# irap-omp/deconv3d

Measured on AMD Instinct MI355X. Metric: spaxel-updates/sec (MH-Gibbs), higher is better.
Workload: dtype f64; 1 GPU; c3_300x300x128; fsf=moffat 11x11, lsf_taps=17, spaxels=90000, lsf=analytic MUSE stand-in (mpdaf absent), parallelism=1 chain, variance=per-voxel cube (heteroscedastic)

## Files before the change

__graft_entry__.py:

```python
import os
import subprocess
import sys

ROOT = os.path.dirname(os.path.abspath(__file__))
if ROOT not in sys.path:
    sys.path.insert(0, ROOT)
CSRC = os.path.join(ROOT, "deconv3d_amd", "csrc")


SOURCES = ["d3d_api.hip", "d3d_spatial.hip", "d3d_mh.hip", "d3d_sweep.hip", "d3d_post.hip", "d3d_region.hip", "d3d_search.hip", "d3d_prep.hip", "d3d_temper.hip", "d3d_robust.hip", "d3d_pred.hip", "d3d_noise.hip", "d3d_ctx.h", "d3d_kernels.h", "d3d_conv.h",
           "d3d_mh_small.h", "d3d_rng.h", "../../include/deconv3d_hip.h", "d3d_strips.h"]


def tree_source_hash():
    import hashlib
    h = hashlib.sha256()
    for name in SOURCES:
        with open(os.path.join(CSRC, name), "rb") as f:
            h.update(f.read())
    return h.hexdigest()[:16]


def _binary_hash(lib):
    code = ("import ctypes,sys; l=ctypes.CDLL(sys.argv[1]); "
            "l.d3d_source_hash.restype=ctypes.c_char_p; print(l.d3d_source_hash().decode())")
    try:
        return subprocess.check_output([sys.executable, "-c", code, lib],
                                       stderr=subprocess.DEVNULL).decode().strip()
    except (subprocess.CalledProcessError, OSError):
        return None


def build():
    env = dict(os.environ)
    lib = os.path.join(CSRC, "libdeconv3d_hip.so")
    want = tree_source_hash()
    have = _binary_hash(lib) if os.path.exists(lib) else None
    fresh = have != want or env.get("D3D_FORCE_REBUILD") == "1"
    cmd = ["make", "-C", CSRC, "-j4", "ARCH=gfx950"] + (["-B"] if fresh else [])
    subprocess.check_call(cmd, env=env)
    if not os.path.exists(lib):
        raise RuntimeError("build did not produce %s" % lib)
    have = _binary_hash(lib)
    if have != want:
        raise RuntimeError("libdeconv3d_hip.so reports source hash %s, the tree has %s" % (have, want))
    print("build: libdeconv3d_hip.so %s (source hash %s)"
          % ("compiled with hipcc --offload-arch=gfx950" if fresh else "up to date", want))
    import deconv3d_amd
    from deconv3d_amd import _lib
    handle = _lib.load()
    missing = [s for s in _lib.SYMBOLS if not hasattr(handle, s)]
    if missing:
        raise RuntimeError("libdeconv3d_hip.so lacks symbols: %s" % missing)


def smoke():
    import numpy as np

    from deconv3d_amd import _lib
    from oracle import deconv3d_oracle as O

    if _lib.device_count() < 1:
        raise RuntimeError("smoke() needs a HIP device (cuda:0); there is no CPU fallback")
    D, H, W = 32, 16, 16
# ... 30 lines not shown
```

deconv3d_amd/csrc/d3d_api.hip:

```cpp
#include "d3d_ctx.h"

#include <dlfcn.h>

#define D3D_VERSION 300
#ifndef D3D_SOURCE_HASH
#define D3D_SOURCE_HASH "unknown"
#endif

namespace {
thread_local std::string g_err;
}

namespace d3dh {
int fail(int code, const char *fmt, ...) {
    char buf[512];
    va_list ap;
    va_start(ap, fmt);
    vsnprintf(buf, sizeof buf, fmt, ap);
    va_end(ap);
    g_err = buf;
    return code;
}
}

// ... 163 lines not shown
                        if (!is_real) list.push_back(make_int4(y, x, 0, 0));
                    }
                if (pt.real[col] > 0) {
                    const long n_all_col =
                        ((long)list.size() - pt.off[col]) * (c->mh_zb ? (c->Dp + 255) / 256 : 1);
                    if (c->mh_zigzag && (ord & 1) && n_all_col > c->flow_grid) {
                        std::reverse(list.begin() + pt.off[col], list.begin() + pt.off[col] + pt.real[col]);
                        std::reverse(list.begin() + pt.off[col] + pt.real[col], list.end());
                    }
                    ++ord;
                }
                most = std::max(most, (int)list.size() - pt.off[col]);
            }
        pt.off[ncol] = (int)list.size();
        const long most_wgs = (long)most * (c->mh_zb ? (c->Dp + 255) / 256 : 1);
        pt.layers = (!c->mh_layers_forced && most_wgs < c->flow_grid / 2) ? 1 : c->mh_layers_cfg;
        const bool partitioned = c->tiled || !c->part_rects.empty();
        pt.wide = pt.layers == 1 && c->mh_wide && partitioned && c->Dp == 128 && most > 0 &&
                  most <= c->flow_grid / 4 && c->mh_defer == 1;
        pt.small = pt.layers == 1 && most_wgs < c->flow_grid / 2;
        pt.strips = 1;
        pt.soff.clear();
        pt.sreal.clear();
        {
            const bool uv = c->ivar_is_uniform && c->uniform_fast_path;
            const int want = c->mh_strips_opt >= 2 ? c->mh_strips_opt
                             : (c->mh_strips_opt == 0 && most_wgs >= c->flow_grid / 2 && !uv) ? MH_STRIPS_AUTO : 1;
            d3d_strips::Plan plan;
            if (want >= 2 && !empty && !partitioned && c->mh_defer == 1 && (c->Dp <= d3d::MH_WS_MAX_DP || c->mh_zb) &&
                !d3dh::mh_part_uses_tables(c, pt) && !c->mh_chain_opt && !c->mh_flow && !c->mh_pair &&
                d3d_strips::plan(c->H, c->fh, want, &plan)) {
                pt.strips = plan.S;
                pt.soff.assign((size_t)ncol * (plan.S + 1), 0);
                pt.sreal.assign((size_t)ncol * plan.S, 0);
                for (int col = 0; col < ncol; ++col) {
                    const int cy = col / c->fw;
                    auto key = [&](const int4 &e) {
                        return 2 * d3d_strips::strip_of_row(plan, d3d_strips::lattice_row(e.x, cy, c->fh)) + (e.z ? 0 : 1);
                    };
                    const auto b = list.begin() + pt.off[col], e = list.begin() + pt.off[col + 1];
                    for (auto it = b; it != e; ++it)
                        if (key(*it) < 0) return fail(D3D_ERR_HIP, "internal: lattice row outside the strips");
                    std::stable_sort(b, e, [&](const int4 &p, const int4 &q) { return key(p) < key(q); });
                    int *so = &pt.soff[(size_t)col * (plan.S + 1)];
                    for (auto it = b; it != e; ++it) {
                        const int k = key(*it);
                        ++so[k / 2 + 1];
                        if (!(k & 1)) ++pt.sreal[(size_t)col * plan.S + k / 2];
                    }
                    for (int s = 0; s < plan.S; ++s) so[s + 1] += so[s];
                }
            }
        }
        pt.chain = false;
        pt.K = 0;
        pt.last_col = -1;
        for (int col = 0; col < ncol; ++col)
            if (pt.real[col] > 0) {
                ++pt.K;
                pt.last_col = col;
            }
#ifdef D3D_EXPERIMENTS
        if (!empty && pt.K > 0) {
            const int cus = c->flow_grid / 4;
            const int fhh_ = (c->fh - 1) / 2, fhw_ = (c->fw - 1) / 2;
            const int lx0 = ((0 - c->gx0) % c->fw + c->fw) % c->fw;
            pt.chain_sx0 = (pt.dx0 - fhw_) - ((((pt.dx0 - fhw_) - lx0) % c->fw + c->fw) % c->fw);
            pt.n_sy = (pt.dy1 - pt.dy0 + 2 * c->fh - 2) / c->fh;
            pt.n_sx = (pt.dx1 + fhw_ - 1 - pt.chain_sx0) / c->fw + 1;
            (void)fhh_;
            pt.chain_ns = c->fw * c->HL;
            const int nt = (pt.chain_ns + 63) / 64 * 64 + 64;
            const bool fh_ok = c->fh == 3 || c->fh == 5 || c->fh == 7 || c->fh == 9 || c->fh == 11;
            const double g_bytes = 4.0 * pt.K * pt.n_sy * pt.n_sx * c->Dp * 8.0;
            const size_t lds = d3d::mh_chain_lds_doubles(c->fw, c->Dp, c->N, ncol, pt.K, nt / 64 - 1) * 8;
            pt.chain = c->mh_chain_opt == 1 && c->mh_defer == 1 && c->Dp <= 256 && pt.layers == 1 &&
                       (long)pt.n_sy * pt.n_sx <= cus && fh_ok && c->fw >= 3 && nt <= MH_CHAIN_NT &&
                       c->Dp <= pt.chain_ns && lds <= (size_t)160 * 1024 && g_bytes <= 512e6 &&
                       c->cube_elems * sizeof(double) < (size_t(1) << 31);
        }
#endif
    }
    {
        size_t need_slots = 0, need_G = 0;
        std::vector<int2> cols((size_t)c->parts.size() * ncol, make_int2(0, 0));
        bool any = false;
        for (size_t pi = 0; pi < c->parts.size(); ++pi) {
            const d3d_ctx::Part &pt = c->parts[pi];
            if (!pt.chain) continue;
            any = true;
            need_slots = std::max(need_slots, (size_t)pt.n_sy * pt.n_sx);
            need_G = std::max(need_G, (size_t)4 * pt.K * pt.n_sy * pt.n_sx * c->Dp);
            int k = 0;
            for (int col = 0; col < ncol; ++col)
                if (pt.real[col] > 0)
                    cols[pi * ncol + k++] = make_int2(((col / c->fw - c->gy0) % c->fh + c->fh) % c->fh,
                                                      ((col % c->fw - c->gx0) % c->fw + c->fw) % c->fw);
        }
        if (any) {
            HIP_TRY(c->chain_cols.reserve(cols.size()));
            HIP_TRY(hipMemcpyAsync(c->chain_cols, cols.data(), cols.size() * sizeof(int2),
                                   hipMemcpyHostToDevice, c->stream));
            if (2 * need_slots > c->chain_flags.size()) {
                HIP_TRY(c->chain_flags.alloc(2 * need_slots));
                HIP_TRY(hipMemsetAsync(c->chain_flags, 0, 2 * need_slots * sizeof(unsigned), c->stream));
                c->chain_base = 0;
// ... 127 lines not shown
        (void)hipGetLastError();
        c->rescale = {};
        return fail(D3D_ERR_HIP, "the base 1/variance (a cube of %zu bytes): %s", bytes, hipGetErrorString(e));
    }
    c->rescale.who = who;
    c->rescale.every = every;
    c->rescale.start = start;
    c->rescale.was_uniform = c->ivar_is_uniform;
    c->ivar_is_uniform = false;
    return 0;
}

void d3dh::rescale_disarm(d3d_ctx *c, d3d_ctx::Rescale::Who who) {
    if (!who || c->rescale.who != who) return;
    (void)hipMemcpyAsync(c->slot[D3D_SLOT_IVAR], c->rescale.i0, c->cube_elems * sizeof(double), hipMemcpyDeviceToDevice,
                         c->stream);
    (void)hipStreamSynchronize(c->stream);
    c->ivar_is_uniform = c->rescale.was_uniform;
    c->rescale = {};
}

bool d3dh::rescale_due(const d3d_ctx *c, int s) {
    if (!c->rescale.who) return false;
    const int64_t rs = (int64_t)s + (int64_t)c->sweep_origin;
    return rs >= c->rescale.start && (rs - c->rescale.start) % c->rescale.every == 0;
}

int d3dh::rescale_after_sweep(d3d_ctx *c, int s) {
    if (!rescale_due(c, s)) return 0;
    const int64_t rs = (int64_t)s + (int64_t)c->sweep_origin;
    return c->rescale.who == d3d_ctx::Rescale::ROBUST ? robust_draw(c, rs) : noise_draw(c, rs);
}

namespace {

enum OptKind { OPT_LAUNCH = 0, OPT_MH = 1, OPT_TAPS = 2 };
struct OptDesc {
    const char *key, *env;
    int d3d_ctx::*field;
    OptKind kind;
    int lo, hi;
};
const OptDesc g_opts[] = {
    {"mh_defer", "D3D_MH_DEFER", &d3d_ctx::mh_defer_opt, OPT_MH, 0, 2},
    {"mh_zblocks", "D3D_MH_ZBLOCKS", &d3d_ctx::mh_zblocks, OPT_MH, 0, 1},
    {"mh_layers", "D3D_MH_LAYERS", &d3d_ctx::mh_layers_opt, OPT_MH, 0, d3d::MH_LAYERS},
    {"mh_wide", "D3D_MH_WIDE", &d3d_ctx::mh_wide, OPT_MH, 0, 1},
    {"mh_props", "D3D_MH_PROPS", &d3d_ctx::mh_props, OPT_LAUNCH, 0, 1},
    {"mh_small", "D3D_MH_SMALL", &d3d_ctx::mh_small, OPT_MH, 0, 2},
    {"halo_timing", "D3D_HALO_TIMING", &d3d_ctx::halo_timing, OPT_LAUNCH, 0, 1},
    {"mh_zigzag", "D3D_MH_ZIGZAG", &d3d_ctx::mh_zigzag, OPT_MH, 0, 1},
    {"mh_nt_ivar", "D3D_MH_NT_IVAR", &d3d_ctx::mh_nt_ivar_opt, OPT_MH, -1, 1},
    {"mh_strips", "D3D_MH_STRIPS", &d3d_ctx::mh_strips_opt, OPT_MH, 0, d3d_strips::MAX_STRIPS},
    {"mh_nt", "D3D_MH_NT", &d3d_ctx::mh_nt_opt, OPT_MH, 0, 1024},
    {"uniform_ivar", "D3D_UNIFORM_IVAR", &d3d_ctx::uniform_fast_path, OPT_MH, 0, 1},
    {"conv_rows", "D3D_CONV_ROWS", &d3d_ctx::conv_rows, OPT_LAUNCH, 0, 1},
    {"conv_zb", "D3D_CONV_ZB", &d3d_ctx::conv_zb, OPT_LAUNCH, 0, 1},
    {"conv_hy", "D3D_CONV_HY", &d3d_ctx::conv_hy_opt, OPT_LAUNCH, 0, 1 << 20},
    {"spatial_sep", "D3D_SPATIAL_SEP", &d3d_ctx::spatial_sep, OPT_TAPS, 0, 1},
    {"sep_fuse", "D3D_SEP_FUSE", &d3d_ctx::sep_fuse, OPT_LAUNCH, 0, 1},
    {"spatial_mode", "D3D_SPATIAL_MODE", &d3d_ctx::march_mode, OPT_LAUNCH, 0, 3},
    {"march_hy", "D3D_MARCH_HY", &d3d_ctx::march_hy_opt, OPT_TAPS, 0, 1 << 20},
    {"zmajor", "D3D_ZMAJOR", &d3d_ctx::zmajor, OPT_LAUNCH, 0, 1},
    {"zmajor_hy", "D3D_ZMAJOR_HY", &d3d_ctx::zmajor_hy, OPT_LAUNCH, 0, 1 << 20},
    {"spectral_dense", "D3D_SPECTRAL_DENSE", &d3d_ctx::spectral_dense, OPT_LAUNCH, 0, 1},
    {"spectral_blocks", "D3D_SPECTRAL_BLOCKS", &d3d_ctx::spectral_blocks, OPT_LAUNCH, 0, 1},
    {"lines_dense", "D3D_LINES_DENSE", &d3d_ctx::lines_dense, OPT_LAUNCH, 0, 3},
    {"lines_rounds", "D3D_LINES_ROUNDS", &d3d_ctx::lines_rounds, OPT_LAUNCH, 0, 64},
    {"spatial_nt", "D3D_SPATIAL_NT", &d3d_ctx::sp_nt_opt, OPT_LAUNCH, 0, 1024},
    {"xcd_remap", "D3D_XCD_REMAP", &d3d_ctx::xcd_remap, OPT_LAUNCH, 0, 1},
    {"alt_dir", "D3D_ALT_DIR", &d3d_ctx::alt_dir, OPT_LAUNCH, 0, 1},
    {"stagger", "D3D_STAGGER", &d3d_ctx::stagger, OPT_LAUNCH, 0, 1 << 20},
    {"post_nt", "D3D_POST_NT", &d3d_ctx::post_nt, OPT_LAUNCH, 0, 1},
    {"noise_timing", "D3D_NOISE_TIMING", &d3d_ctx::noise_timing, OPT_LAUNCH, 0, 1},
#ifdef D3D_EXPERIMENTS
    {"mh_chain", "D3D_MH_CHAIN", &d3d_ctx::mh_chain_opt, OPT_MH, 0, 1},
    {"mh_prio", "D3D_MH_PRIO", &d3d_ctx::mh_prio, OPT_LAUNCH, 0, 255},
    {"mh_maxit", "D3D_MH_MAXIT", &d3d_ctx::mh_maxit_opt, OPT_MH, -1, 32},
    {"mh_flow", "D3D_MH_FLOW", &d3d_ctx::mh_flow, OPT_MH, 0, 1},
    {"mh_pair", "D3D_MH_PAIR", &d3d_ctx::mh_pair, OPT_MH, 0, 1},
    {"spectral_shfl", "D3D_SPECTRAL_SHFL", &d3d_ctx::spectral_shfl, OPT_LAUNCH, 0, 1},
    {"fuse_lsf", "D3D_FUSE_LSF", &d3d_ctx::fuse_lsf, OPT_TAPS, 0, 1},
    {"march_pf", "D3D_MARCH_PF", &d3d_ctx::march_pf, OPT_LAUNCH, 0, 3},
    {"march_one", "D3D_MARCH_ONE", &d3d_ctx::march_one, OPT_LAUNCH, 0, 3},
    {"march_stamp", "D3D_STAMP", &d3d_ctx::march_stamp, OPT_LAUNCH, 0, 1},
#endif
};

const OptDesc *find_opt(const char *key) {
    for (const OptDesc &o : g_opts)
        if (!strcmp(o.key, key)) return &o;
    return nullptr;
}

bool opt_value_ok(const OptDesc &o, long v) {
    if (v < o.lo || v > o.hi) return false;
    if (!strcmp(o.key, "mh_nt")) return v == 0 || v == 128 || v == 256 || v == 512 || v == 1024;
    if (!strcmp(o.key, "spatial_nt")) return v == 0 || v == 256 || v == 512 || v == 1024;
    if (!strcmp(o.key, "mh_maxit")) return v == -1 || v == 0 || v == 4 || v == 8 || v == 16 || v == 32;
    return true;
}

void options_from_env(d3d_ctx *c) {
    for (const OptDesc &o : g_opts)
        if (const char *e = getenv(o.env)) {
            const long v = atol(e);
// ... 111 lines not shown
        CTX_TRY(c->gbuf[b].alloc((size_t)c->slots * c->Dp));
        CTX_TRY(hipMemsetAsync(c->gbuf[b], 0, (size_t)c->slots * c->Dp * sizeof(double), c->stream));
    }
    {
#ifdef D3D_EXPERIMENTS
        const size_t ncol = (size_t)fh * fw;
        c->flow_LY = H / fh + 3;
        c->flow_LX = W / fw + 3;
        c->flow_cap_K = ncol;
        c->flow_cap_items = c->spx.size();
        CTX_TRY(c->flow_ent.alloc(c->spx.size()));
        CTX_TRY(c->flow_col.alloc(ncol));
        CTX_TRY(c->flow_lat.alloc(ncol * c->flow_LY * c->flow_LX));
        c->flow_state_bytes = ((4 + ncol + c->spx.size()) * sizeof(unsigned) + 15) / 16 * 16;
        CTX_TRY(c->flow_state.alloc(c->flow_state_bytes / sizeof(unsigned)));
        CTX_TRY(c->pair_state.alloc((4 + c->spx.size())));
        CTX_TRY(hipMemsetAsync(c->pair_state, 0, (4 + c->spx.size()) * sizeof(unsigned), c->stream));
#endif
        CTX_TRY(c->flow_err.alloc(4));
        CTX_TRY(hipMemsetAsync(c->flow_err, 0, 16, c->stream));
        int cus = 0;
        CTX_TRY(hipDeviceGetAttribute(&cus, hipDeviceAttributeMultiprocessorCount, device));
        c->flow_grid = 4 * (cus > 0 ? cus : 256);
    }
    CTX_TRY(hipMemsetAsync(c->dlog, 0, (size_t)c->HW * sizeof(double), c->stream));
    CTX_TRY(hipMemsetAsync(c->accepted, 0, sizeof(unsigned long long), c->stream));
    CTX_TRY(hipMemsetAsync(c->acc_map, 0, (size_t)c->HW * sizeof(unsigned), c->stream));
    CTX_TRY(hipMemsetAsync(c->mask, 1, (size_t)c->HW, c->stream));
    CTX_TRY(hipStreamSynchronize(c->stream));
#undef CTX_TRY
    c->h_mask.assign((size_t)c->HW, 1);
    c->h_user_mask.assign((size_t)c->HW, 1);
    *out = c;
    return D3D_OK;
}

int d3d_ctx_destroy(d3d_ctx *c) {
    if (!c) return D3D_OK;
    (void)hipSetDevice(c->device);
    if (c->stream) (void)hipStreamSynchronize(c->stream);
    if (c->comm && g_rccl.CommDestroy) (void)g_rccl.CommDestroy(c->comm);
    c->comm = nullptr;
    for (int b = 0; b < d3d_ctx::STREAM_NB; ++b) {
        if (c->snap_host[b]) (void)hipHostFree(c->snap_host[b]);
        if (c->snap_ready[b]) (void)hipEventDestroy(c->snap_ready[b]);
        if (c->snap_done[b]) (void)hipEventDestroy(c->snap_done[b]);
    }
    if (c->copy_stream) (void)hipStreamDestroy(c->copy_stream);
    for (int a = 0; a < d3d_ctx::STRIP_AUX; ++a) {
        if (c->strip_stream[a]) (void)hipStreamDestroy(c->strip_stream[a]);
        if (c->strip_join[a]) (void)hipEventDestroy(c->strip_join[a]);
    }
    if (c->strip_fork) (void)hipEventDestroy(c->strip_fork);
    for (hipEvent_t e : c->halo_ev) (void)hipEventDestroy(e);
    if (c->ev0) (void)hipEventDestroy(c->ev0);
    if (c->ev1) (void)hipEventDestroy(c->ev1);
    if (c->own_stream) (void)hipStreamDestroy(c->own_stream);
    delete c;
    return D3D_OK;
}

int d3d_ctx_set_stream(d3d_ctx *c, void *hip_stream) {
    NEED(c, D3D_ERR_INVALID, "ctx is NULL");
    HIP_TRY(hipStreamSynchronize(c->stream));
    c->stream = hip_stream ? (hipStream_t)hip_stream : c->own_stream;
    return D3D_OK;
}

int d3d_sync(d3d_ctx *c) {
    NEED(c, D3D_ERR_INVALID, "ctx is NULL");
    HIP_TRY(hipStreamSynchronize(c->stream));
    return D3D_OK;
}

int d3d_timer_start(d3d_ctx *c) {
    NEED(c, D3D_ERR_INVALID, "ctx is NULL");
    HIP_TRY(hipEventRecord(c->ev0, c->stream));
    return D3D_OK;
}

int d3d_timer_stop(d3d_ctx *c, double *ms) {
    NEED(c && ms, D3D_ERR_INVALID, "NULL argument");
    HIP_TRY(hipEventRecord(c->ev1, c->stream));
    HIP_TRY(hipEventSynchronize(c->ev1));
    float f = 0.f;
    HIP_TRY(hipEventElapsedTime(&f, c->ev0, c->ev1));
    *ms = (double)f;
    return D3D_OK;
}

static int set_taps_impl(d3d_ctx *c, const double *fsf, const double *lsf, double thr);

int d3d_set_taps(d3d_ctx *c, const double *fsf, const double *lsf, double thr) {
    NEED(c && fsf, D3D_ERR_INVALID, "NULL argument");
    c->h_fsf.assign(fsf, fsf + (size_t)c->fh * c->fw);
    c->h_has_lsf = lsf != nullptr;
    if (lsf) c->h_lsf.assign(lsf, lsf + c->D);
    c->h_thr = thr;
    if (int rc = set_taps_impl(c, c->h_fsf.data(), c->h_has_lsf ? c->h_lsf.data() : nullptr, thr)) return rc;
    return post_reset(c);
}

int d3d_ctx_set_option(d3d_ctx *c, const char *key, long value) {
    NEED(c && key, D3D_ERR_INVALID, "NULL argument");
    const OptDesc *o = find_opt(key);
    NEED(o, D3D_ERR_INVALID, "unknown option '%s'", key);
// ... 2 lines not shown
    HIP_TRY(hipSetDevice(c->device));
    if (c->adapt.on && value != 0 &&
        (!strcmp(key, "mh_chain") || !strcmp(key, "mh_flow") || !strcmp(key, "mh_pair")))
        return fail(D3D_ERR_UNSUPPORTED,
                    "option %s with per-spaxel jump scales on (d3d_adapt_begin): the kernel keeps its "
                    "proposals' inputs across sweeps", key);
    if (c->prior.on && value != 0 &&
        (!strcmp(key, "mh_chain") || !strcmp(key, "mh_flow") || !strcmp(key, "mh_pair")))
        return fail(D3D_ERR_UNSUPPORTED,
                    "option %s with the smoothness prior on (d3d_prior_begin): the kernel decides more "
                    "than one colour class in a launch", key);
    if (o->kind == OPT_MH)
        if (int rc = flush_pending(c)) return rc;
    c->*(o->field) = (int)value;
    if (o->kind == OPT_MH) {
        pick_mh_geometry(c);
        if (c->have_data) return build_colour_lists(c);
    } else if (o->kind == OPT_TAPS && c->have_taps) {
        return set_taps_impl(c, c->h_fsf.data(), c->h_has_lsf ? c->h_lsf.data() : nullptr, c->h_thr);
    }
    return D3D_OK;
}

int d3d_ctx_get_option(d3d_ctx *c, const char *key, long *value) {
    NEED(c && key && value, D3D_ERR_INVALID, "NULL argument");
    if (!strcmp(key, "chain_parts")) {
        long n = 0;
        for (const d3d_ctx::Part &pt : c->parts) n += pt.chain ? 1 : 0;
        *value = c->have_data ? n : 0;
        return D3D_OK;
    }
    if (!strcmp(key, "search_bank_ns") || !strcmp(key, "search_kernel_ns")) {
        *value = key[7] == 'b' ? c->search_bank_ns : c->search_kernel_ns;
        return D3D_OK;
    }
    if (!strcmp(key, "prep_median_ns") || !strcmp(key, "prep_stats_ns")) {
        *value = key[5] == 'm' ? c->prep_median_ns : c->prep_stats_ns;
        return D3D_OK;
    }
    if (!strcmp(key, "noise_sums_ns") || !strcmp(key, "noise_draw_ns") || !strcmp(key, "noise_apply_ns")) {
        *value = c->noise_ns[key[6] == 's' ? 0 : key[6] == 'd' ? 1 : 2];
        return D3D_OK;
    }
    if (!strcmp(key, "device_bytes")) {
        *value = (long)d3dh::dev_bytes.load();
        return D3D_OK;
    }
    if (!strcmp(key, "mh_nt_ivar_on")) {
        *value = c->mh_nt_ivar ? 1 : 0;
        return D3D_OK;
    }
    if (!strcmp(key, "mh_strips_on")) {
        *value = (c->have_data && c->parts.size() == 1 && c->parts[0].strips > 1) ? c->parts[0].strips : 0;
        return D3D_OK;
    }
    if (!strcmp(key, "mh_path")) {
        *value = c->mh_path.code;
        return D3D_OK;
    }
    if (!strcmp(key, "mh_path_layers")) {
        *value = (long)c->mh_path.layers;
        return D3D_OK;
    }
    if (!strcmp(key, "mh_path_launches")) {
        *value = c->mh_path.launches;
        c->mh_path = {};
        return D3D_OK;
    }
    if (!strcmp(key, "device_cus")) {
        *value = c->flow_grid / 4;
        return D3D_OK;
    }
    if (!strcmp(key, "batch_layers")) {
        *value = c->batch_layers;
        return D3D_OK;
    }
    if (!strcmp(key, "lsf_fits")) {
        *value = (c->have_taps && (c->ntaps == 0 || c->lsf_dense_any)) ? 1 : 0;
        return D3D_OK;
    }
    if (!strcmp(key, "lsf_taps")) {
        *value = c->ntaps;
        return D3D_OK;
    }
    if (!strcmp(key, "spatial_path") || !strcmp(key, "spectral_path") || !strcmp(key, "stage_path")) {
        *value = key[2] == 'a' ? (key[3] == 't' ? c->spatial_path : c->stage_path) : c->spectral_path;
        return D3D_OK;
    }
    if (!strcmp(key, "small_parts")) {
        long n = 0;
        for (const d3d_ctx::Part &pt : c->parts) n += d3dh::mh_part_uses_tables(c, pt) ? 1 : 0;
        *value = c->have_data ? n : 0;
        return D3D_OK;
    }
    const OptDesc *o = find_opt(key);
    NEED(o, D3D_ERR_INVALID, "unknown option '%s'", key);
    *value = c->*(o->field);
    return D3D_OK;
}

int d3d_has_experiments(void) {
#ifdef D3D_EXPERIMENTS
    return 1;
#else
    return 0;
#endif
// ... 1290 lines not shown
```

deconv3d_amd/csrc/d3d_ctx.h:

```cpp
#pragma once
#include <hip/hip_runtime.h>
#include <rccl/rccl.h>

#include <algorithm>
#include <atomic>
#include <cmath>
#include <cstdarg>
#include <cstdio>
#include <cstdlib>
#include <cstring>
#include <mutex>
#include <new>
#include <string>
#include <utility>
#include <vector>

#include "../../include/deconv3d_hip.h"
#include "d3d_kernels.h"
#include "d3d_strips.h"

#ifndef D3D_WIDE_NS
#define D3D_WIDE_NS 704
#endif
constexpr int MH_WIDE_NS = D3D_WIDE_NS;
constexpr int MH_CHAIN_NT = 768;
constexpr int MH_STRIPS_AUTO = 2;

namespace d3dh {
int fail(int code, const char *fmt, ...);
}

#define HIP_TRY(expr)                                                                   \
    do {                                                                                \
        hipError_t e_ = (expr);                                                         \
        if (e_ != hipSuccess)                                                           \
            return d3dh::fail(D3D_ERR_HIP, "%s failed: %s (%s:%d)", #expr, hipGetErrorString(e_), \
                              __FILE__, __LINE__);                                      \
    } while (0)

#define NEED(cond, code, ...) \
    do {                      \
        if (!(cond)) return d3dh::fail(code, __VA_ARGS__); \
    } while (0)

namespace d3dh {
inline std::atomic<size_t> dev_bytes{0};
}

template <typename T>
class DevBuf {
    T *p_ = nullptr;
    size_t n_ = 0;

   public:
    DevBuf() = default;
    DevBuf(DevBuf &&o) noexcept : p_(std::exchange(o.p_, nullptr)), n_(std::exchange(o.n_, 0)) {}
    DevBuf &operator=(DevBuf &&o) noexcept {
        std::swap(p_, o.p_);
        std::swap(n_, o.n_);
        o.reset();
        return *this;
    }
    ~DevBuf() { reset(); }
    hipError_t alloc(size_t n) {
        reset();
        const hipError_t e = hipMalloc(&p_, n * sizeof(T));
        if (e != hipSuccess) {
            p_ = nullptr;
            return e;
        }
        n_ = n;
        d3dh::dev_bytes += n * sizeof(T);
        return e;
    }
    hipError_t reserve(size_t n) { return n <= n_ ? hipSuccess : alloc(n); }
    void reset() {
        if (p_) (void)hipFree(p_);
        d3dh::dev_bytes -= n_ * sizeof(T);
        p_ = nullptr;
        n_ = 0;
    }
    T *get() const { return p_; }
    operator T *() const { return p_; }
    size_t size() const { return n_; }
};

struct d3d_ctx {
    int device = 0;
    int D = 0, H = 0, W = 0, fh = 0, fw = 0;
    int Dp = 0, HL = 0, N = 0;
    bool deep = false;
    long HW = 0;
    size_t cube_elems = 0;
    hipStream_t own_stream = nullptr, stream = nullptr;
    hipEvent_t ev0 = nullptr, ev1 = nullptr;

    DevBuf<double> slot[D3D_SLOT_COUNT];
    DevBuf<double> stage;
    DevBuf<double> stage2;
    DevBuf<double> params;
    DevBuf<double> params_alt;
    DevBuf<uint8_t> mask;
    DevBuf<double> fsf;
    DevBuf<int> lsf_shift;
    DevBuf<double> lsf_weight;
    int ntaps = 0;
    DevBuf<double> dlog;
    DevBuf<double> hwbuf;
    DevBuf<double> scal;
    DevBuf<unsigned long long> accepted;
    DevBuf<unsigned> acc_map;
    DevBuf<int4> spx;
    std::vector<int> colour_real;
    struct Part {
        int y0 = 0, y1 = 0, x0 = 0, x1 = 0;
        int dy0 = 0, dy1 = 0, dx0 = 0, dx1 = 0;
        int phase = 0;
        int layers = 1;
        bool wide = false;
        bool small = false;
        bool chain = false;
        int chain_ns = 0, chain_sx0 = 0, n_sy = 0, n_sx = 0, K = 0;
        int last_col = -1;
        std::vector<int> off;
        std::vector<int> real;
        int strips = 1;
        std::vector<int> soff;
        std::vector<int> sreal;
    };
    std::vector<Part> parts;
    std::vector<int4> part_rects;
    std::vector<int> part_phase;
    int n_phases = 1;
    int pend_part = -1;
    struct HaloEntry {
        int peer = 0, what = 0;
        int sy0 = 0, sy1 = 0, sx0 = 0, sx1 = 0;
        int ry0 = 0, ry1 = 0, rx0 = 0, rx1 = 0;
        size_t send_off = 0, send_n = 0, recv_off = 0, recv_n = 0;
    };
    std::vector<std::vector<HaloEntry>> plans;
    DevBuf<double> halo_send, halo_recv;
    static constexpr int STREAM_NB = 4;
    hipStream_t copy_stream = nullptr;
    DevBuf<double> snap_dev[STREAM_NB];
    double *snap_host[STREAM_NB] = {};
    hipEvent_t snap_ready[STREAM_NB] = {}, snap_done[STREAM_NB] = {};
    static constexpr int STRIP_AUX = 3;
    hipStream_t strip_stream[STRIP_AUX] = {};
    hipEvent_t strip_fork = nullptr, strip_join[STRIP_AUX] = {};
    int mh_strips_opt = 0;
    ncclComm_t comm = nullptr;
    int comm_rank = -1, comm_size = 0;
    int halo_timing = 0;
    static constexpr size_t HALO_RING = 64;
    std::vector<hipEvent_t> halo_ev;
    size_t halo_ev_used = 0, halo_ev_head = 0;
    double halo_ms = 0.0;
    long halo_count = 0;
    std::vector<uint8_t> h_mask;
    std::vector<uint8_t> h_user_mask;

    d3d::LineShape line = {1, {0.0, 0.0, 0.0, 0.0}, {1.0, 0.0, 0.0, 0.0}, nullptr, 0, 0.0, 0.0};
    DevBuf<double> line_tab;
    std::vector<double> h_line_tab;
    double line_tab_flux = 0.0;
    bool have_taps = false, have_data = false, have_params = false, have_cfg = false;
    bool err_valid = false;
    double min_b[3] = {}, max_b[3] = {}, amp[3] = {};
    double ra = 0;
    uint64_t seed = 0;
    int refresh_every = 1000;
    uint32_t sweep_origin = 0;

    int mh_nt = 0, mh_maxit = 0;
    int mh_nt_opt = 0, mh_maxit_opt = -1;
    int mh_defer = 1;
    int mh_defer_opt = 1;
    int mh_zblocks = 1;
    bool mh_zb = false;
    DevBuf<double> z_part;
    DevBuf<double> z_E;
#ifdef D3D_EXPERIMENTS
    DevBuf<unsigned long long> stampbuf;
    size_t stamp_launches = 0, stamp_next = 0, stamp_stride = 0;
#endif
    bool ivar_is_uniform = false;
    double ivar_uniform = 0.0;
    int uniform_fast_path = 1;
    static constexpr int GBUFS = 8;
    DevBuf<double> gbuf[GBUFS];
    int lay_n = 0, lay_cy[3] = {-1, -1, -1}, lay_cx[3] = {-1, -1, -1}, lay_g[3] = {0, 0, 0};
    int mh_layers = 2;
    int batch_layers = 0;
    bool mh_nt_ivar = false;
    int mh_nt_ivar_opt = -1;
    int mh_zigzag = 1;
    int mh_layers_opt = 0;
    int mh_layers_cfg = 2;
    bool mh_layers_forced = false;
    int mh_flow = 0;
    int flow_K = 0, flow_LY = 0, flow_LX = 0, flow_items = 0, flow_grid = 0;
    int flow_last_cy = -1, flow_last_cx = -1;
    int mh_chain_opt = 0;
// ... 266 lines not shown
```

deconv3d_amd/csrc/d3d_sweep.hip:

```cpp
#include "d3d_ctx.h"

using namespace d3dh;

void d3dh::colour_residue(const d3d_ctx *c, int col, int *cy, int *cx) {
    *cy = ((col / c->fw - c->gy0) % c->fh + c->fh) % c->fh;
    *cx = ((col % c->fw - c->gx0) % c->fw + c->fw) % c->fw;
}

namespace {

struct SnapQueue {
    int slot[d3d_ctx::STREAM_NB];
    int head = 0, count = 0;
};

int snap_setup(d3d_ctx *c) {
    if (c->copy_stream) return 0;
    HIP_TRY(hipStreamCreateWithFlags(&c->copy_stream, hipStreamNonBlocking));
    const size_t bytes = (size_t)c->HW * 4 * sizeof(double);
    for (int b = 0; b < d3d_ctx::STREAM_NB; ++b) {
        HIP_TRY(c->snap_dev[b].alloc((size_t)c->HW * 4));
        HIP_TRY(hipHostMalloc((void **)&c->snap_host[b], bytes, hipHostMallocDefault));
        HIP_TRY(hipEventCreateWithFlags(&c->snap_ready[b], hipEventDisableTiming));
        HIP_TRY(hipEventCreateWithFlags(&c->snap_done[b], hipEventDisableTiming));
// ... 39 lines not shown
    HIP_TRY(hipSetDevice(c->device));
    if (!c->err_valid)
        if (int rc = d3d_residual(c, nullptr)) return rc;
    if (zero_accepted) {
        HIP_TRY(hipMemsetAsync(c->accepted, 0, sizeof(unsigned long long), c->stream));
        HIP_TRY(hipMemsetAsync(c->acc_map, 0, (size_t)c->HW * sizeof(unsigned), c->stream));
    }
    c->props_sweep = -1;
    return 0;
}

int active_ordinal(const d3d_ctx::Part &pt, int col) {
    int ord = 0;
    for (int k = 0; k < col; ++k) ord += pt.real[k] > 0;
    return ord;
}

void fill_colour_args(d3d_ctx *c, const d3d_ctx::Part &pt, int col, int ka, int layers, int tables,
                      d3d::MHArgs &P) {
    fill_mh_args(c, P);
    P.spx = c->spx + pt.off[col];
    P.rev = (c->mh_zigzag && (ka & 1)) ? 1 : 0;
    if (tables) P.props = c->props;
    if (tables > 1) {
        P.ltab = c->ltab;
        P.ptab = c->ptab;
        int ly, lx;
        colour_residue(c, col, &ly, &lx);
        for (int j = 0; j < 2; ++j) P.ptab_row[j] = mh_ptab_row(c, ly, lx, j);
    }
    if (layers) P.write_back = (c->lay_n >= layers) ? 1 : 0;
}

void push_colour_layer(d3d_ctx *c, int pi, int col, int g, bool wrote_back) {
    if (wrote_back) c->lay_n = 0;
    int cy, cx;
    colour_residue(c, col, &cy, &cx);
    pend_push(c, cy, cx, g);
    c->pend_part = pi;
}

int launch_real(d3d_ctx *c, const d3d_ctx::Part &pt, int col, const d3d::MHArgs &P, uint32_t sweep) {
    if (pt.strips <= 1) return launch_mh(c, P, (unsigned)pt.real[col], sweep);
    for (int s = 0; s < pt.strips; ++s) {
        const int n = pt.sreal[(size_t)col * pt.strips + s];
        if (n <= 0) continue;
        d3d::MHArgs Ps = P;
        Ps.spx = P.spx + pt.soff[(size_t)col * (pt.strips + 1) + s];
        if (int rc = launch_mh(c, Ps, (unsigned)n, sweep)) return rc;
    }
    return 0;
}

struct StripScope {
    d3d_ctx *c;
    hipStream_t main;
    int S = 1, row = -1;
    unsigned locked = 0;
    int setup() {
        if (c->strip_fork) return 0;
        for (int b = 4; b < d3d_ctx::GBUFS; ++b) {
            HIP_TRY(c->gbuf[b].alloc((size_t)c->slots * c->Dp));
            HIP_TRY(hipMemsetAsync(c->gbuf[b], 0, (size_t)c->slots * c->Dp * sizeof(double), main));
        }
        HIP_TRY(hipEventCreateWithFlags(&c->strip_fork, hipEventDisableTiming));
        for (int a = 0; a < d3d_ctx::STRIP_AUX; ++a) {
            HIP_TRY(hipStreamCreateWithFlags(&c->strip_stream[a], hipStreamNonBlocking));
            HIP_TRY(hipEventCreateWithFlags(&c->strip_join[a], hipEventDisableTiming));
        }
        return 0;
    }
    int free_buf() const {
        for (int b = 0; b < d3d_ctx::GBUFS; ++b) {
            bool used = (locked >> b) & 1;
            for (int j = 0; j < c->lay_n; ++j) used = used || c->lay_g[j] == b;
            if (!used) return b;
        }
        return 0;
    }
    int fork(int strips, int colour_row, unsigned locked_bufs) {
        if (int rc = setup()) return rc;
        locked = locked_bufs;
        HIP_TRY(hipEventRecord(c->strip_fork, main));
        for (int a = 0; a + 1 < strips; ++a) HIP_TRY(hipStreamWaitEvent(c->strip_stream[a], c->strip_fork, 0));
        S = strips;
        row = colour_row;
        return 0;
    }
    int join() {
        c->stream = main;
        const int n = S;
        S = 1;
        row = -1;
        locked = 0;
        for (int a = 0; a + 1 < n; ++a) {
            HIP_TRY(hipEventRecord(c->strip_join[a], c->strip_stream[a]));
            HIP_TRY(hipStreamWaitEvent(main, c->strip_join[a], 0));
        }
        return 0;
    }
    ~StripScope() { (void)join(); }
};

struct Batch {
    d3d_ctx **cs;
    int R, layers;
    bool small;
    const d3d::MHChainArgs *dev;
};

int run_part(d3d_ctx *c, int pi, uint32_t sweep, const Batch *b = nullptr, bool strips_allowed = false) {
    d3d_ctx::Part &pt = c->parts[pi];
    const int ncol = c->fh * c->fw;
    const int layers = b ? b->layers : pt.layers;
    d3d_ctx *const self[1] = {c};
    d3d_ctx *const *cs = b ? b->cs : self;
    const bool partitioned = c->tiled || c->parts.size() > 1;
    const bool deferred =
        c->mh_defer &&
        (!partitioned || (c->mh_defer == 1 && (c->Dp <= d3d::MH_WS_MAX_DP || c->mh_zb)));
    if (c->lay_n && (c->pend_part != pi || !deferred || c->lay_n > layers))
        if (int rc = flush_pending(c)) return rc;
#ifdef D3D_EXPERIMENTS
    if (deferred && pt.chain && !b) return launch_mh_chain(c, pi, sweep, 1);
#endif
    const bool pairs = !b && deferred && c->mh_pair && !partitioned && c->mh_defer == 1 && c->Dp <= 256 &&
                       pt.layers == 2 && c->flow_K > 1 && !c->flow_first.empty();
    const bool small = deferred && c->mh_defer == 1 && !c->mh_zb && d3dh::mh_part_uses_tables(c, pt);
    const int tables = b ? (b->small ? 2 : 0)
                         : (c->mh_props && deferred && (c->mh_zb || (pt.layers == 1 && !c->deep) || small))
                               ? (small ? 2 : 1) : 0;
    bool strips_ok = strips_allowed && !b && pt.strips > 1 && deferred && !partitioned && c->mh_defer == 1 && tables < 2 &&
                     (c->mh_zb || c->Dp <= d3d::MH_WS_MAX_DP);
#ifdef D3D_EXPERIMENTS
    strips_ok = strips_ok && !c->stampbuf && !pairs;
#endif
    StripScope strips = {c, c->stream};
    int ord = 0;
    for (int col = 0; col < ncol; ++col) {
        const int n_real = pt.real[col];
        if (n_real <= 0) continue;
        const int ka = ord++;
        if (deferred) c->pend_part = pi;
#ifdef D3D_EXPERIMENTS
        if (pairs && c->lay_n == 1 && ka + 1 < c->flow_K) {
            if (c->stampbuf) goto single;
            int rc = launch_mh_pair(c, ka, sweep);
            if (rc) return rc;
            ++col;
            while (col < ncol && pt.real[col] <= 0) ++col;
            ++ord;
            continue;
        }
    single:
#else
        (void)pairs;
#endif
        if (tables && !b)
            if (int rc = ensure_proposals(c, sweep)) return rc;
        d3d::MHArgs P;
        fill_colour_args(c, pt, col, ka, deferred ? layers : 0, tables, P);
        if (!deferred) {
            if (int rc = launch_real(c, pt, col, P, sweep)) return rc;
            continue;
        }
        const int n_all = pt.off[col + 1] - pt.off[col];
        if (strips.S > 1 && col / c->fw != strips.row)
            if (int rc = strips.join()) return rc;
        if (strips_ok && strips.S == 1) {
            int cy, cx;
            colour_residue(c, col, &cy, &cx);
            unsigned locked = 0;
            for (int j = 0; j < c->lay_n; ++j)
                if (c->lay_cy[j] != cy) locked |= 1u << c->lay_g[j];
            if (int rc = strips.fork(pt.strips, col / c->fw, locked)) return rc;
        }
        if (strips.S > 1) {
            const int g_cur = strips.free_buf();
            P.Gcur = c->gbuf[g_cur];
            const int *so = &pt.soff[(size_t)col * (pt.strips + 1)];
            for (int s = 0; s < pt.strips; ++s) {
                const int n = so[s + 1] - so[s];
                if (n <= 0) continue;
                d3d::MHArgs Ps = P;
                Ps.spx = P.spx + so[s];
                c->stream = s ? c->strip_stream[s - 1] : strips.main;
                const int rc = c->mh_zb ? launch_mh_zb(c, Ps, (unsigned)n, sweep, layers, (unsigned)n_all, (unsigned)s)
                                        : launch_mh_defer(c, Ps, (unsigned)n, sweep, layers, pt.wide, (unsigned)n_all);
                c->stream = strips.main;
                if (rc) return rc;
            }
            push_colour_layer(c, pi, col, g_cur, P.write_back);
            continue;
        }
#ifdef D3D_EXPERIMENTS
        if (!b && c->stampbuf && c->stamp_next < c->stamp_launches && (size_t)n_all * 8 <= c->stamp_stride)
            P.stamp = c->stampbuf + (c->stamp_next++) * c->stamp_stride;
#endif
        const int g_cur = pend_free_buf(c);
        int rc;
        if (b) {
            P.batch = b->dev;
            P.b_items = n_all;
            P.b_gcur = g_cur;
            for (int j = 0; j < 3; ++j) P.b_lay_g[j] = j < c->lay_n ? c->lay_g[j] : 0;
            rc = launch_mh_batch(c, P, (unsigned)n_all * b->R, sweep, layers);
        } else {
            rc = c->mh_zb ? launch_mh_zb(c, P, (unsigned)n_all, sweep, layers)
                          : launch_mh_defer(c, P, (unsigned)n_all, sweep, layers, pt.wide);
        }
        if (rc) return rc;
        for (int r = 0; r < (b ? b->R : 1); ++r) push_colour_layer(cs[r], pi, col, g_cur, P.write_back);
    }
    return strips.join();
}

int run_phase(d3d_ctx *c, int phase, uint32_t sweep, bool strips_allowed = false) {
    for (size_t pi = 0; pi < c->parts.size(); ++pi)
        if (c->parts[pi].phase == phase)
            if (int rc = run_part(c, (int)pi, sweep, nullptr, strips_allowed)) return rc;
    return 0;
}

int end_sweep(d3d_ctx *c, int s, int keep_one_in, SnapQueue &snaps, double *chain_out, double *dlog_out) {
    if (s % keep_one_in == 0 && (chain_out || dlog_out))
        if (int rc = snap_push(c, snaps, s / keep_one_in, chain_out, dlog_out)) return rc;
    if (post_due(c, s))
        if (int rc = post_sample(c)) return rc;
    if (int rc = adapt_after_sweep(c, s)) return rc;
    if (c->refresh_every > 0 && s % c->refresh_every == 0) {
        if (plan_has_entries(c, D3D_PLAN_PARAMS)) {
            NEED(c->comm, D3D_ERR_STATE, "parameter gather needs d3d_comm_init");
            if (int rc = halo_exchange(c, D3D_PLAN_PARAMS)) return rc;
        }
        if (int rc = forward_into(c, c->slot[D3D_SLOT_ERR], true)) return rc;
    }
    return rescale_after_sweep(c, s);
}

int halo_drain_one(d3d_ctx *c) {
    const size_t at = c->halo_ev_head;
    float f = 0.f;
    HIP_TRY(hipEventSynchronize(c->halo_ev[2 * at + 1]));
    HIP_TRY(hipEventElapsedTime(&f, c->halo_ev[2 * at], c->halo_ev[2 * at + 1]));
    c->halo_ms += (double)f;
// ... 251 lines not shown
```

Baseline: 19.68 million spaxel-updates/s.

## Replace per-row strip fork/join with neighbour-only event schedule across colour rows

Adds a precomputed strip schedule in which each strip stream, at the start of a new colour row, waits only on events from its adjacent strips instead of a full join to the main stream and a fresh fork. G buffers are assigned from two alternating pools so a row can start while the previous row's layers are still pending. The aim is to remove global fork/join barriers between colour rows and let strips run ahead independently. In exchange it adds more event records and waits per colour, a more complex buffer-rotation scheme that must stay correct, and an optional lag-injection kernel for testing.

```diff
diff --git a/__graft_entry__.py b/__graft_entry__.py
--- a/__graft_entry__.py
+++ b/__graft_entry__.py
@@ -9,7 +9,7 @@
 
 
 SOURCES = ["d3d_api.hip", "d3d_spatial.hip", "d3d_mh.hip", "d3d_sweep.hip", "d3d_post.hip", "d3d_region.hip", "d3d_search.hip", "d3d_prep.hip", "d3d_temper.hip", "d3d_robust.hip", "d3d_pred.hip", "d3d_noise.hip", "d3d_ctx.h", "d3d_kernels.h", "d3d_conv.h",
-           "d3d_mh_small.h", "d3d_rng.h", "../../include/deconv3d_hip.h", "d3d_strips.h"]
+           "d3d_mh_small.h", "d3d_rng.h", "../../include/deconv3d_hip.h", "d3d_strips.h", "d3d_strip_order.h"]
 
 
 def tree_source_hash():
diff --git a/deconv3d_amd/csrc/d3d_api.hip b/deconv3d_amd/csrc/d3d_api.hip
--- a/deconv3d_amd/csrc/d3d_api.hip
+++ b/deconv3d_amd/csrc/d3d_api.hip
@@ -239,6 +239,13 @@
                 }
             }
         }
+        pt.order = d3d_strip_order::Schedule();
+        if (pt.strips > 1 && (c->mh_strip_order_opt ? c->mh_strip_order_opt : MH_STRIP_ORDER_AUTO) == 2) {
+            std::vector<int> active;
+            for (int col = 0; col < ncol; ++col)
+                if (pt.real[col] > 0) active.push_back(col);
+            (void)d3d_strip_order::build(pt.strips, c->fw, active, pt.layers, &pt.order);
+        }
         pt.chain = false;
         pt.K = 0;
         pt.last_col = -1;
@@ -472,6 +479,8 @@
     {"mh_zigzag", "D3D_MH_ZIGZAG", &d3d_ctx::mh_zigzag, OPT_MH, 0, 1},
     {"mh_nt_ivar", "D3D_MH_NT_IVAR", &d3d_ctx::mh_nt_ivar_opt, OPT_MH, -1, 1},
     {"mh_strips", "D3D_MH_STRIPS", &d3d_ctx::mh_strips_opt, OPT_MH, 0, d3d_strips::MAX_STRIPS},
+    {"mh_strip_order", "D3D_MH_STRIP_ORDER", &d3d_ctx::mh_strip_order_opt, OPT_MH, 0, 2},
+    {"mh_strip_lag", "D3D_MH_STRIP_LAG", &d3d_ctx::mh_strip_lag, OPT_LAUNCH, 0, d3d_strips::MAX_STRIPS},
     {"mh_nt", "D3D_MH_NT", &d3d_ctx::mh_nt_opt, OPT_MH, 0, 1024},
     {"uniform_ivar", "D3D_UNIFORM_IVAR", &d3d_ctx::uniform_fast_path, OPT_MH, 0, 1},
     {"conv_rows", "D3D_CONV_ROWS", &d3d_ctx::conv_rows, OPT_LAUNCH, 0, 1},
@@ -689,6 +698,8 @@
         if (c->strip_join[a]) (void)hipEventDestroy(c->strip_join[a]);
     }
     if (c->strip_fork) (void)hipEventDestroy(c->strip_fork);
+    for (hipEvent_t e : c->strip_ev)
+        if (e) (void)hipEventDestroy(e);
     for (hipEvent_t e : c->halo_ev) (void)hipEventDestroy(e);
     if (c->ev0) (void)hipEventDestroy(c->ev0);
     if (c->ev1) (void)hipEventDestroy(c->ev1);
@@ -797,6 +808,11 @@
     }
     if (!strcmp(key, "mh_strips_on")) {
         *value = (c->have_data && c->parts.size() == 1 && c->parts[0].strips > 1) ? c->parts[0].strips : 0;
+        return D3D_OK;
+    }
+    if (!strcmp(key, "mh_strip_order_on")) {
+        const bool strips = c->have_data && c->parts.size() == 1 && c->parts[0].strips > 1;
+        *value = !strips ? 0 : c->parts[0].order.S > 1 ? 2 : 1;
         return D3D_OK;
     }
     if (!strcmp(key, "mh_path")) {
diff --git a/deconv3d_amd/csrc/d3d_ctx.h b/deconv3d_amd/csrc/d3d_ctx.h
--- a/deconv3d_amd/csrc/d3d_ctx.h
+++ b/deconv3d_amd/csrc/d3d_ctx.h
@@ -17,6 +17,7 @@
 
 #include "../../include/deconv3d_hip.h"
 #include "d3d_kernels.h"
+#include "d3d_strip_order.h"
 #include "d3d_strips.h"
 
 #ifndef D3D_WIDE_NS
@@ -25,6 +26,7 @@
 constexpr int MH_WIDE_NS = D3D_WIDE_NS;
 constexpr int MH_CHAIN_NT = 768;
 constexpr int MH_STRIPS_AUTO = 2;
+constexpr int MH_STRIP_ORDER_AUTO = 2;
 
 namespace d3dh {
 int fail(int code, const char *fmt, ...);
@@ -127,6 +129,7 @@
         int strips = 1;
         std::vector<int> soff;
         std::vector<int> sreal;
+        d3d_strip_order::Schedule order;
     };
     std::vector<Part> parts;
     std::vector<int4> part_rects;
@@ -150,6 +153,11 @@
     hipStream_t strip_stream[STRIP_AUX] = {};
     hipEvent_t strip_fork = nullptr, strip_join[STRIP_AUX] = {};
     int mh_strips_opt = 0;
+    hipEvent_t strip_ev[d3d_strip_order::NEV] = {};
+    int strip_gbuf[d3d_strip_order::GSLOTS] = {0, 1, 2, 3, 4, 5, 6, 7};
+    int strip_pool = 0;
+    int mh_strip_order_opt = 0;
+    int mh_strip_lag = 0;
     ncclComm_t comm = nullptr;
     int comm_rank = -1, comm_size = 0;
     int halo_timing = 0;
diff --git a/deconv3d_amd/csrc/d3d_strip_order.h b/deconv3d_amd/csrc/d3d_strip_order.h
--- /dev/null
+++ b/deconv3d_amd/csrc/d3d_strip_order.h
@@ -0,0 +1,95 @@
+#pragma once
+
+#include <vector>
+
+#include "d3d_strips.h"
+
+namespace d3d_strip_order {
+
+constexpr int MAX_STRIPS = d3d_strips::MAX_STRIPS;
+constexpr int MAX_LAYERS = 3;
+constexpr int GSLOTS = 2 * (MAX_LAYERS + 1);
+
+constexpr int EV_FORK = 0;
+constexpr int ev_down(int s) { return s; }
+constexpr int ev_up(int s) { return MAX_STRIPS + s; }
+constexpr int ev_join(int s) { return 2 * MAX_STRIPS - 1 + s; }
+constexpr int NEV = 3 * MAX_STRIPS - 1;
+
+struct Step {
+    int col = 0;
+    int row = 0;
+    bool first_of_row = false;
+    int pool = 0, gidx = 0;
+    unsigned pre[MAX_STRIPS] = {};
+    unsigned wait[MAX_STRIPS] = {};
+    unsigned post[MAX_STRIPS] = {};
+};
+
+struct Schedule {
+    int S = 0, M = 0, rows = 0;
+    std::vector<Step> steps;
+    unsigned tail_post[MAX_STRIPS] = {};
+    unsigned tail_wait[MAX_STRIPS] = {};
+};
+
+inline int gslot(const Schedule &sd, const Step &st, int pool0) { return ((st.pool ^ pool0) & 1) * (sd.M + 1) + st.gidx; }
+inline int pool_after(const Schedule &sd, int pool0) { return (pool0 ^ sd.rows) & 1; }
+
+inline bool build(int S, int fw, const std::vector<int> &colours, int M, Schedule *out) {
+    *out = Schedule();
+    if (S < 2 || S > MAX_STRIPS || M < 1 || M > MAX_LAYERS || fw < 1 || colours.empty()) return false;
+    Schedule sd;
+    const int n = (int)colours.size();
+    sd.steps.resize(n);
+    int row = -1, in_row = 0, last_cr = -1;
+    for (int k = 0; k < n; ++k) {
+        if (colours[k] < 0 || (k && colours[k] <= colours[k - 1])) return false;
+        const int cr = colours[k] / fw;
+        if (cr != last_cr) {
+            if (row >= 0 && in_row < M) return false;
+            ++row;
+            in_row = 0;
+            last_cr = cr;
+        }
+        Step &st = sd.steps[k];
+        st.col = colours[k];
+        st.row = row;
+        st.first_of_row = in_row == 0;
+        st.pool = row & 1;
+        st.gidx = in_row % (M + 1);
+        ++in_row;
+    }
+    if (in_row < M) return false;
+    sd.rows = row + 1;
+    for (int k = 0; k < n; ++k) {
+        Step &st = sd.steps[k];
+        if (k == 0) {
+            st.pre[0] |= 1u << EV_FORK;
+            for (int s = 1; s < S; ++s) st.wait[s] |= 1u << EV_FORK;
+        }
+        const bool last_of_row = k + 1 == n || sd.steps[k + 1].row != st.row;
+        const bool more_rows = st.row + 1 < sd.rows;
+        int ord = 0;
+        for (int j = k; j > 0 && sd.steps[j - 1].row == st.row; --j) ++ord;
+        if (more_rows && last_of_row)
+            for (int s = 1; s < S; ++s) st.post[s] |= 1u << ev_down(s);
+        if (more_rows && ord == M - 1)
+            for (int s = 0; s + 1 < S; ++s) st.post[s] |= 1u << ev_up(s);
+        if (st.first_of_row && st.row > 0)
+            for (int s = 0; s < S; ++s) {
+                if (s + 1 < S) st.wait[s] |= 1u << ev_down(s + 1);
+                if (s > 0) st.wait[s] |= 1u << ev_up(s - 1);
+            }
+    }
+    for (int s = 1; s < S; ++s) {
+        sd.tail_post[s] |= 1u << ev_join(s);
+        sd.tail_wait[0] |= 1u << ev_join(s);
+    }
+    sd.S = S;
+    sd.M = M;
+    *out = sd;
+    return true;
+}
+
+}
diff --git a/deconv3d_amd/csrc/d3d_sweep.hip b/deconv3d_amd/csrc/d3d_sweep.hip
--- a/deconv3d_amd/csrc/d3d_sweep.hip
+++ b/deconv3d_amd/csrc/d3d_sweep.hip
@@ -115,6 +115,13 @@
     return 0;
 }
 
+static_assert(d3d_ctx::GBUFS == d3d_strip_order::GSLOTS, "a G buffer behind every slot of the schedule");
+
+__global__ __launch_bounds__(64) void k_strip_lag() {
+    const uint64_t t0 = wall_clock64();
+    for (int i = 0; i < 40 && wall_clock64() - t0 < 10000; ++i) __builtin_amdgcn_s_sleep(127);
+}
+
 struct StripScope {
     d3d_ctx *c;
     hipStream_t main;
@@ -150,8 +157,79 @@
         row = colour_row;
         return 0;
     }
+    const d3d_strip_order::Schedule *sched = nullptr;
+    int pool0 = 0;
+    hipStream_t stream_of(int s) const { return s ? c->strip_stream[s - 1] : main; }
+    int record(unsigned mask, int s) {
+        for (int e = 0; e < d3d_strip_order::NEV; ++e)
+            if ((mask >> e) & 1) HIP_TRY(hipEventRecord(c->strip_ev[e], stream_of(s)));
+        return 0;
+    }
+    int wait(unsigned mask, int s) {
+        for (int e = 0; e < d3d_strip_order::NEV; ++e)
+            if ((mask >> e) & 1) HIP_TRY(hipStreamWaitEvent(stream_of(s), c->strip_ev[e], 0));
+        return 0;
+    }
+    int enter(const d3d_strip_order::Schedule &sd, int k) {
+        namespace so = d3d_strip_order;
+        const so::Step &st = sd.steps[(size_t)k];
+        if (k == 0) {
+            if (int rc = setup()) return rc;
+            for (int e = 0; e < so::NEV; ++e)
+                if (!c->strip_ev[e]) HIP_TRY(hipEventCreateWithFlags(&c->strip_ev[e], hipEventDisableTiming));
+            pool0 = c->strip_pool & 1;
+            const int other = (1 - pool0) * (sd.M + 1);
+            bool placed = true;
+            for (int j = 0; j < c->lay_n; ++j) {
+                bool in = false;
+                for (int q = 0; q <= sd.M; ++q) in = in || c->strip_gbuf[other + q] == c->lay_g[j];
+                placed = placed && in;
+            }
+            if (!placed) {
+                int order[d3d_ctx::GBUFS], n = 0;
+                for (int j = 0; j < c->lay_n; ++j) order[n++] = c->lay_g[j];
+                for (int b = 0; b < d3d_ctx::GBUFS; ++b) {
+                    bool pending = false;
+                    for (int j = 0; j < c->lay_n; ++j) pending = pending || c->lay_g[j] == b;
+                    if (!pending) order[n++] = b;
+                }
+                n = 0;
+                for (int q = 0; q <= sd.M; ++q) c->strip_gbuf[other + q] = order[n++];
+                for (int q = 0; q <= sd.M; ++q) c->strip_gbuf[pool0 * (sd.M + 1) + q] = order[n++];
+                for (int q = 2 * (sd.M + 1); q < so::GSLOTS; ++q) c->strip_gbuf[q] = order[n++];
+            }
+            c->strip_pool = so::pool_after(sd, pool0);
+            S = sd.S;
+            sched = &sd;
+        }
+        for (int s = 0; s < sd.S; ++s)
+            if (int rc = record(st.pre[s], s)) return rc;
+        for (int s = 0; s < sd.S; ++s)
+            if (int rc = wait(st.wait[s], s)) return rc;
+        if (st.first_of_row && c->mh_strip_lag >= 1 && c->mh_strip_lag <= sd.S) {
+            hipLaunchKernelGGL(k_strip_lag, dim3(1), dim3(64), 0, stream_of(c->mh_strip_lag - 1));
+            HIP_TRY(hipGetLastError());
+        }
+        return 0;
+    }
+    int buf_of(int k) const { return c->strip_gbuf[d3d_strip_order::gslot(*sched, sched->steps[(size_t)k], pool0)]; }
+    int leave(int k) {
+        for (int s = 0; s < sched->S; ++s)
+            if (int rc = record(sched->steps[(size_t)k].post[s], s)) return rc;
+        return 0;
+    }
     int join() {
         c->stream = main;
+        if (sched) {
+            const d3d_strip_order::Schedule &sd = *sched;
+            sched = nullptr;
+            S = 1;
+            for (int s = 0; s < sd.S; ++s)
+                if (int rc = record(sd.tail_post[s], s)) return rc;
+            for (int s = 0; s < sd.S; ++s)
+                if (int rc = wait(sd.tail_wait[s], s)) return rc;
+            return 0;
+        }
         const int n = S;
         S = 1;
         row = -1;
@@ -228,18 +306,7 @@
             continue;
         }
         const int n_all = pt.off[col + 1] - pt.off[col];
-        if (strips.S > 1 && col / c->fw != strips.row)
-            if (int rc = strips.join()) return rc;
-        if (strips_ok && strips.S == 1) {
-            int cy, cx;
-            colour_residue(c, col, &cy, &cx);
-            unsigned locked = 0;
-            for (int j = 0; j < c->lay_n; ++j)
-                if (c->lay_cy[j] != cy) locked |= 1u << c->lay_g[j];
-            if (int rc = strips.fork(pt.strips, col / c->fw, locked)) return rc;
-        }
-        if (strips.S > 1) {
-            const int g_cur = strips.free_buf();
+        auto launch_strips = [&](int g_cur) {
             P.Gcur = c->gbuf[g_cur];
             const int *so = &pt.soff[(size_t)col * (pt.strips + 1)];
             for (int s = 0; s < pt.strips; ++s) {
@@ -254,6 +321,29 @@
                 if (rc) return rc;
             }
             push_colour_layer(c, pi, col, g_cur, P.write_back);
+            return 0;
+        };
+        if (strips_ok && pt.order.S > 1) {
+            NEED(pt.order.S == pt.strips && pt.order.M == layers && ka < (int)pt.order.steps.size() &&
+                     pt.order.steps[(size_t)ka].col == col,
+                 D3D_ERR_STATE, "internal: the strips' schedule does not describe colour %d", col);
+            if (int rc = strips.enter(pt.order, ka)) return rc;
+            if (int rc = launch_strips(strips.buf_of(ka))) return rc;
+            if (int rc = strips.leave(ka)) return rc;
+            continue;
+        }
+        if (strips.S > 1 && col / c->fw != strips.row)
+            if (int rc = strips.join()) return rc;
+        if (strips_ok && strips.S == 1) {
+            int cy, cx;
+            colour_residue(c, col, &cy, &cx);
+            unsigned locked = 0;
+            for (int j = 0; j < c->lay_n; ++j)
+                if (c->lay_cy[j] != cy) locked |= 1u << c->lay_g[j];
+            if (int rc = strips.fork(pt.strips, col / c->fw, locked)) return rc;
+        }
+        if (strips.S > 1) {
+            if (int rc = launch_strips(strips.free_buf())) return rc;
             continue;
         }
 #ifdef D3D_EXPERIMENTS
```

After: 20.44 million spaxel-updates/s, median of 6. 3.9% higher.
